# clearmatics/libff

Measured on AMD Instinct MI355X. Metric: G1 MSM throughput (scalar-muls/sec), higher is better.
Workload: dtype u32

## Files before the change

### libff_amd/csrc/group_vtable.h

```cpp
#pragma once
#include <hip/hip_runtime_api.h>
#include <stddef.h>
#include <stdint.h>
#include <stdlib.h>

namespace amdmsm {

enum out_form : int {
    OUT_JACOBIAN = 0,
    OUT_LIBFF = 1,
    OUT_AFFINE = 2,
};

struct sort_geom {
    int hb;
    int fb;
    uint32_t chunk_cap;
    uint32_t big_thresh;
    uint32_t big_cap;
    size_t big_words;
};
constexpr int SORT_HB_MAX = 10;
constexpr size_t SORT_COARSE_WORDS = ((size_t)1 << SORT_HB_MAX) + 1, SORT_CURSOR_WORDS = (size_t)1 << SORT_HB_MAX;
inline sort_geom sort_geometry(size_t n, int c, int W) {
// ... 98 lines not shown
    int fr_words;
    int el_words;
    int fq_words;
    int fr_bits;
    int projective;
    int reduce_fold;
    int bucket_words;
    const uint32_t* fr_one_mont;
    const uint32_t* fr_modulus;
    int has_endomorphism;
    int coeff_a_nonzero;
    int glv_bound_log2_x1000;
    int prime_order;
    const uint32_t* glv_lambda;

    void (*import_bases)(hipStream_t, const uint32_t* src, size_t stride_words, int form_special,
                         size_t n, uint32_t* dst_affine);
    void (*export_affine)(hipStream_t, const uint32_t* src_affine, size_t n, uint32_t* dst_xyz);
    void (*gen_bases_seq)(hipStream_t, unsigned long long first, size_t n, uint32_t* dst_affine);
    void (*endo_points)(hipStream_t, const uint32_t* bases_affine, size_t n, uint32_t* out);
    void (*precompute_table)(hipStream_t, const uint32_t* bases_affine, size_t n, int c, int D, uint32_t* tmp,
                             uint32_t* table);
    void (*ffi_decode_points)(hipStream_t, const uint32_t* src_be, size_t n, uint32_t* dst_affine, uint32_t* status);
    void (*ffi_decode_scalars)(hipStream_t, const uint32_t* src_be, size_t n, uint32_t* dst_plain, uint32_t* status);
    void (*ffi_encode_point)(hipStream_t, const uint32_t* src_xyz_affine, uint32_t* dst_be);
    void (*disk_decode)(hipStream_t, const uint32_t* src, size_t n, uint32_t* dst_affine);
    void (*disk_decode_compressed)(hipStream_t, const uint32_t* src, size_t n, uint32_t* dst_affine, uint32_t* status);
    void (*disk_encode)(hipStream_t, const uint32_t* src_affine, size_t n, uint32_t* dst);
    void (*disk_encode_compressed)(hipStream_t, const uint32_t* src_affine, size_t n, uint32_t* dst);

    void (*scalar_stats)(hipStream_t, const uint32_t* scalars, size_t n, int mont, uint32_t* stats);
    void (*scalar_bits)(hipStream_t, const void* scalars, int kind, size_t n, int mont, uint32_t* out_bits);
    void (*gather_scalars)(hipStream_t, const uint32_t* shared, size_t shared_n, const uint32_t* index, size_t offset,
                           uint32_t* flag, size_t n, uint32_t* out);
    void (*count)(hipStream_t, const uint32_t* scalars, size_t n, int mont, int c, int W, uint32_t* counts);
    void (*scatter)(hipStream_t, const uint32_t* scalars, size_t n, int mont, int c, int W, uint32_t* cursor,
                    uint32_t* lists, size_t list_stride);
    void (*sort)(hipStream_t, const sort_src& src, size_t n, int mont, int c, int W, const sort_bufs& bufs, int mode);
    int (*sort_top_window)(int mode, int mont, int c, int W, size_t columns, int* tb);

    void (*accumulate)(hipStream_t, const uint32_t* ends, const uint32_t* lists, size_t list_stride,
                       const uint32_t* bases_affine, uint32_t* buckets, uint32_t* part_first, uint32_t* part_last,
                       uint32_t* cont_bucket, int W, uint32_t B, uint32_t S, uint32_t T, const uint32_t* endo_points,
                       size_t n_real, int overlap);
    size_t (*accumulate_resident_lanes)(int overlap);
    int accumulate_overlap_ok;
    void (*accumulate_fixup)(hipStream_t, const uint32_t* ends, uint32_t* buckets, uint32_t* part_first,
                             const uint32_t* part_last, const uint32_t* cont_bucket, uint32_t* queue, int W,
                             uint32_t B, uint32_t S, uint32_t T);

    void (*reduce_segments)(hipStream_t, const uint32_t* buckets, int W, uint32_t B, uint32_t L, uint32_t* out);
    void (*sum_butterfly)(hipStream_t, const uint32_t* in, int W, uint32_t M, uint32_t* out);
    void (*sum_block)(hipStream_t, const uint32_t* in, int W, uint32_t M, uint32_t* out);
    void (*reduce_rowcol)(hipStream_t, const uint32_t* buckets, int W, uint32_t B, int c, uint32_t q_row, uint32_t q_col,
                          uint32_t* rc, uint32_t* planes, uint32_t* out);
    void (*horner)(hipStream_t, const uint32_t* window_sums, int W, int c, int form, const uint32_t* init,
                   uint32_t* out);
    void (*horner_batch)(hipStream_t, const uint32_t* window_sums, int k, int W, int c, int form, uint32_t* const* outs);
    void (*sum_points)(hipStream_t, const uint32_t* pts, int k, int form, uint32_t* out);

    void (*fixed_base_exp)(hipStream_t, const uint32_t* g_xyz, int scalar_size, int window, const uint32_t* scalars,
                           size_t n, int mont, const uint32_t* coeff, int form, uint32_t* gouter, uint32_t* table,
                           uint32_t* table_aff, int build_table, uint32_t* out);

    int smv_entries;
    void (*smv_table)(hipStream_t, const uint32_t* bases_affine, size_t n, uint32_t* tmp, uint32_t* table);
    void (*smv_ladder)(hipStream_t, const uint32_t* table, size_t n, const uint32_t* scalars, int mont, int form, uint32_t* out);

    int seg_windows, seg_digit_stride;
    void (*seg_digits)(hipStream_t, const uint32_t* scalars, size_t n, int mont, uint32_t* digits);
    void (*seg_accumulate)(hipStream_t, const uint32_t* table, size_t nt, const uint32_t* digits, const uint32_t* slices,
                           size_t n_slices, uint32_t* sums);
    void (*seg_fold)(hipStream_t, const uint32_t* sums, const uint32_t* seg_first, size_t m, uint32_t* winsum);
    void (*seg_horner)(hipStream_t, const uint32_t* winsum, size_t m, int form, uint32_t* out);

    int fold_digit_stride;
    void (*fold_digits)(hipStream_t, const uint32_t* scalars_host, int k, int mont, int glv, int W, uint32_t* digits);
    void (*fold_ladder)(hipStream_t, const uint32_t* tables, size_t n, const uint32_t* digits, int rows, int glv, int W,
                        int form, uint32_t* out);

    void (*fft_gather)(hipStream_t, const uint32_t* in_affine, size_t b0, size_t cn, int rsh, uint32_t* dst_affine);
    void (*fft_butterfly)(hipStream_t, const uint32_t* table, size_t cn, const uint32_t* in_affine, size_t b0, int rsh,
                          const uint32_t* twiddles, int mont, size_t half, uint32_t* out);

    void (*field_op)(hipStream_t, int op, const uint32_t* a, const uint32_t* b, uint32_t* out, size_t n);
    void (*group_op)(hipStream_t, int op, const uint32_t* a, const uint32_t* b, uint32_t* out, size_t n, int form);
    void (*digits)(hipStream_t, const uint32_t* scalars, size_t n, int mont, int c, int W, int32_t* out);
    void (*glv_digits)(hipStream_t, const uint32_t* scalars, size_t n, int mont, int c, int W, int32_t* out);
    void (*mul_bench)(hipStream_t, uint32_t* inout, size_t nthreads, int iters, int inline_variant);
    void (*madd_bench)(hipStream_t, const uint32_t* pts_affine, uint32_t* out_xyz, size_t nthreads, int iters,
                       int inline_variant);

    void (*field_probe)(hipStream_t, int impl, int op, const uint32_t* a, const uint32_t* b, const uint32_t* c,
                        const uint32_t* d, uint32_t* out, uint32_t* flag, size_t n);
    void (*xyzz_probe)(hipStream_t, int impl, int op, const uint32_t* acc, const uint32_t* pt, uint32_t* out, size_t n);
};
constexpr int FOLD_MAX_K = 8;
constexpr size_t FOLD_DIGIT_BYTES = 2048;

enum {
    FPROBE_MUL = 0, FPROBE_SQR = 1, FPROBE_ADD = 2, FPROBE_SUB = 3, FPROBE_NEG = 4, FPROBE_INV = 5, FPROBE_DBL = 6,
    FPROBE_CNEG = 7,
    FPROBE_HALF = 8, FPROBE_TO_MONT = 9, FPROBE_FROM_MONT = 10,
    FPROBE_SQRT = 11,
    FPROBE_MUL_LZ = 16, FPROBE_SQR_LZ = 17, FPROBE_SUB_LZ = 18, FPROBE_ADD_LZ = 19, FPROBE_NEG_LZ = 20,
    FPROBE_MUL_SUB_MUL_LZ = 21,
    FPROBE_IS_ZERO_LZ = 22,
// ... 18 lines not shown
```

### libff_amd/csrc/msm_group.hip

```cpp
#include "curve_params.h"
#include "ec.cuh"
#include "fp2h.cuh"
#include "group_vtable.h"
#include "wide.cuh"
#include "wide28.cuh"
#include "rr.cuh"

#include <algorithm>
#include <cstdio>
#include <vector>
#include <type_traits>

#ifndef AMDMSM_GROUP
#error "compile with -DAMDMSM_GROUP=<group traits> -DAMDMSM_VT=<vtable getter name>"
#endif

namespace amdmsm {
template <bool I>
struct ec_coeff_a<Fp<AMDMSM_GROUP::fq, I>> {
    static constexpr int value = AMDMSM_GROUP::DEG == 1 ? AMDMSM_GROUP::COEFF_A : 0;
};
template <int NR, bool I>
struct ec_coeff_a<Fp2<AMDMSM_GROUP::fq, NR, I>> {
    static constexpr int value = AMDMSM_GROUP::DEG == 2 ? AMDMSM_GROUP::COEFF_A : 0;
// ... 1832 lines not shown
        jac_add(p, p, x);
    }
    wave_group_sum_r(p, RED_FOLD);
    if (lane < (uint32_t)RED_LANES) store_jac(part + wave * XYZW, p);
    __syncthreads();
    if (wave != 0) return;
    const uint32_t jw = lane / RED_LANES;
    if (jw < nw) load_jac(p, part + jw * XYZW); else jac_set_inf(p);
    uint32_t G = 1;
    while (G < nw) G <<= 1;
    wave_group_sum_r(p, G);
    if (lane < (uint32_t)RED_LANES) store_jac(planes + ((size_t)w * c + k) * XYZW, p);
}

__global__ void __launch_bounds__(SUMW_THREADS) k_plane_sums_wide(const uint32_t* __restrict__ rc, int W, int c, int h,
                                                                  uint32_t* __restrict__ planes) {
    __shared__ uint32_t buf[2][SUMW_SLOTS * XYZW];
    __builtin_amdgcn_s_setprio(3);
    const uint32_t w = blockIdx.x / (uint32_t)c, k = blockIdx.x % (uint32_t)c;
    const uint32_t C = 1u << h, R = (1u << (c - 1)) >> h, NP = R + 1 + C;
    const bool from_cols = k < (uint32_t)h;
    const uint32_t* src = rc + ((size_t)w * NP + (from_cols ? R + 1 : 0)) * XYZW;
    const uint32_t bit = from_cols ? k : k - (uint32_t)h;
    const bool top = k == (uint32_t)c - 1;
    const uint32_t M = top ? 1u : (from_cols ? C : R) / 2;
    constexpr uint32_t NLANES = SUMW_THREADS / RED_LANES, NWAVES = SUMW_THREADS / 64;
    const uint32_t i0 = threadIdx.x / RED_LANES, wave = threadIdx.x >> 6;
    Jac<ER> p, x;
    jac_set_inf(p);
    for (uint32_t i = i0; i < M; i += NLANES) {
        const uint32_t idx = top ? R : (((i >> bit) << (bit + 1)) | (1u << bit) | (i & ((1u << bit) - 1u)));
        load_jac(x, src + (size_t)idx * XYZW);
        jac_add(p, p, x);
    }
    wave_group_sum_r(p, 4);
    if ((i0 & 3u) == 0) store_jac(buf[0] + (size_t)(i0 >> 2) * XYZW, p);
    __syncthreads();
    const WideEnv<FQ> env = wide_env<FQ>();
    uint32_t K = ((M < NLANES ? M : NLANES) + 3) / 4;
    int cur = 0;
    while (K > 1) {
        const uint32_t pairs = K / 2;
        for (uint32_t q = wave; q < pairs; q += NWAVES) {
            const uint32_t* a = buf[cur] + (size_t)(2 * q) * XYZW;
            sum_wide_add(env, a, a + XYZW, buf[cur ^ 1] + (size_t)q * XYZW);
        }
        __syncthreads();
        cur ^= 1;
        K = pairs;
    }
    for (uint32_t t = threadIdx.x; t < (uint32_t)XYZW; t += SUMW_THREADS) planes[((size_t)w * c + k) * XYZW + t] = buf[cur][t];
}

template <class P, bool I>
AMDMSM_DEV typename std::enable_if<(P::N < 16), void>::type horner_chain(Jac<Fp<P, I>>& res,
                                                                         const uint32_t* __restrict__ window_sums, int W,
                                                                         int c, const uint32_t* __restrict__ init) {
    const WideEnv<P> env = wide_env<P>();
    auto load = [&](const uint32_t* p, uint32_t& X, uint32_t& Y, uint32_t& Z) {
        X = env.valid ? p[env.j] : 0u;
        Y = env.valid ? p[EW + env.j] : 0u;
        Z = env.valid ? p[2 * EW + env.j] : 0u;
    };
    uint32_t X, Y, Z, X2, Y2, Z2;
    int w = W - 1;
    if (init) {
        load(init, X, Y, Z);
    } else {
        load(window_sums + (size_t)w * XYZW, X, Y, Z);
        --w;
    }
    for (; w >= 0; --w) {
        if (!wide_is_zero(Z)) {
            if constexpr (GP::COEFF_A != 0) for (int i = 0; i < c; ++i) jac_dbl_wide<P, GP::COEFF_A>(env, X, Y, Z);
            else if (c >= 4) jac_dbl_run28<P>(env, X, Y, Z, c);
            else for (int i = 0; i < c; ++i) jac_dbl_wide<P>(env, X, Y, Z);
        }
        load(window_sums + (size_t)w * XYZW, X2, Y2, Z2);
        jac_add_wide<P, GP::COEFF_A>(env, X, Y, Z, X2, Y2, Z2);
    }
    wide_to_packed(res.x, X);
    wide_to_packed(res.y, Y);
    wide_to_packed(res.z, Z);
}
template <class P, bool I>
AMDMSM_DEV typename std::enable_if<(P::N >= 16 && P::N < 32), void>::type horner_chain(
    Jac<Fp<P, I>>& res, const uint32_t* __restrict__ window_sums, int W, int c, const uint32_t* __restrict__ init) {
    using F = WideFq<P>;
    const WideEnv<P> env = wide_env<P>();
    auto load = [&](const uint32_t* p, uint32_t& X, uint32_t& Y, uint32_t& Z) {
        X = env.valid ? p[env.j] : 0u;
        Y = env.valid ? p[EW + env.j] : 0u;
        Z = env.valid ? p[2 * EW + env.j] : 0u;
    };
    uint32_t X, Y, Z, X2, Y2, Z2;
    int w = W - 1;
    if (init) {
        load(init, X, Y, Z);
    } else {
        load(window_sums + (size_t)w * XYZW, X, Y, Z);
        --w;
    }
    for (; w >= 0; --w) {
        if (!wide_is_zero(Z)) {
            if (c >= 4) jac_dbl_run28<P>(env, X, Y, Z, c);
            else for (int i = 0; i < c; ++i) jac_dbl_wide2<P>(env, X, Y, Z);
// ... 94 lines not shown
inline bool horner_lazy() {
    static const bool on = HORNER_LAZY_OK && !(getenv("AMDMSM_HORNER_LAZY") && atoi(getenv("AMDMSM_HORNER_LAZY")) == 0);
    return on;
}

__global__ void __launch_bounds__(64) k_horner(const uint32_t* __restrict__ window_sums, int W, int c, int form,
                                               const uint32_t* __restrict__ init, uint32_t* __restrict__ out) {
    __builtin_amdgcn_s_setprio(3);
    Jac<E> res;
    horner_chain(res, window_sums, W, c, init);
    if (threadIdx.x == 0) store_out(out, res, form);
}
template <class EE = E>
__global__ void __launch_bounds__(64) k_horner_lazy(const uint32_t* __restrict__ window_sums, int W, int c, int form,
                                                    const uint32_t* __restrict__ init, uint32_t* __restrict__ out) {
    __builtin_amdgcn_s_setprio(3);
    Jac<EE> res;
    horner_chain_lazy(res, window_sums, W, c, init);
    if (threadIdx.x == 0) store_out(out, res, form);
}

constexpr int WH_MAX_GROUPS = 6;
__global__ void __launch_bounds__(64 * WH_MAX_GROUPS) k_window_horner(const uint32_t* __restrict__ planes, int c,
                                                                       uint32_t* __restrict__ out) {
    __shared__ uint32_t grp[WH_MAX_GROUPS * XYZW];
    __builtin_amdgcn_s_setprio(3);
    const int wave = (int)(threadIdx.x >> 6), ng = (c + 3) / 4;
    Jac<E> res;
    if (wave < ng) {
        const int k0 = 4 * wave, cnt = (c - k0 < 4) ? c - k0 : 4;
        horner_chain(res, planes + ((size_t)blockIdx.x * c + k0) * XYZW, cnt, 1, nullptr);
        if ((threadIdx.x & 63u) == 0) store_jac(grp + wave * XYZW, res);
    }
    __syncthreads();
    if (wave != 0) return;
    horner_chain(res, grp, ng, 4, nullptr);
    if (threadIdx.x == 0) store_jac(out + (size_t)blockIdx.x * XYZW, res);
}
template <class EE = E>
__global__ void __launch_bounds__(64 * WH_MAX_GROUPS) k_window_horner_lazy(const uint32_t* __restrict__ planes, int c,
                                                                            uint32_t* __restrict__ out) {
    __shared__ uint32_t grp[WH_MAX_GROUPS * XYZW];
    __builtin_amdgcn_s_setprio(3);
    const int wave = (int)(threadIdx.x >> 6), ng = (c + 3) / 4;
    Jac<EE> res;
    if (wave < ng) {
        const int k0 = 4 * wave, cnt = (c - k0 < 4) ? c - k0 : 4;
        horner_chain_lazy(res, planes + ((size_t)blockIdx.x * c + k0) * XYZW, cnt, 1, nullptr);
        if ((threadIdx.x & 63u) == 0) store_jac(grp + wave * XYZW, res);
    }
    __syncthreads();
    if (wave != 0) return;
    horner_chain_lazy(res, grp, ng, 4, nullptr);
    if (threadIdx.x == 0) store_jac(out + (size_t)blockIdx.x * XYZW, res);
}

struct horner_outs {
    uint32_t* p[8];
};
__global__ void __launch_bounds__(64) k_horner_batch(const uint32_t* __restrict__ window_sums, int W, int c, int form,
                                                     horner_outs outs) {
    __builtin_amdgcn_s_setprio(3);
    Jac<E> res;
    horner_chain(res, window_sums + (size_t)blockIdx.x * W * XYZW, W, c, nullptr);
    uint32_t* out = outs.p[0];
#pragma unroll
    for (int j = 1; j < 8; ++j) out = (blockIdx.x == (unsigned)j) ? outs.p[j] : out;
    if (threadIdx.x == 0) store_out(out, res, form);
}
template <class EE = E>
__global__ void __launch_bounds__(64) k_horner_batch_lazy(const uint32_t* __restrict__ window_sums, int W, int c, int form,
                                                          horner_outs outs) {
    __builtin_amdgcn_s_setprio(3);
    Jac<EE> res;
    horner_chain_lazy(res, window_sums + (size_t)blockIdx.x * W * XYZW, W, c, nullptr);
    uint32_t* out = outs.p[0];
#pragma unroll
    for (int j = 1; j < 8; ++j) out = (blockIdx.x == (unsigned)j) ? outs.p[j] : out;
    if (threadIdx.x == 0) store_out(out, res, form);
}

__global__ void __launch_bounds__(64) k_sum_points(const uint32_t* __restrict__ pts, int k, int form,
                                                   uint32_t* __restrict__ out) {
    Jac<E> res;
    if (k <= 0) jac_set_inf(res);
    else horner_chain(res, pts, k, 0, nullptr);
    if (threadIdx.x == 0) store_out(out, res, form);
}

constexpr int IMPORT_K = 32;

__global__ void __launch_bounds__(TPB) k_import_bases(const uint32_t* __restrict__ src, size_t stride_words,
                                                      int form_special, size_t n, uint32_t* __restrict__ dst) {
    if (form_special) {
        const size_t i = gtid();
        if (i >= n) return;
        const uint32_t* q = src + i * stride_words;
        Aff<E> a;
        E z;
        el_load(a.x, q);
        el_load(a.y, q + EW);
        el_load(z, q + 2 * EW);
        if (el_is_zero(z)) {
            el_zero(a.x);
            el_zero(a.y);
        }
// ... 1041 lines not shown

__global__ void __launch_bounds__(TPB) k_seg_fold(const uint32_t* __restrict__ sums, const uint32_t* __restrict__ seg_first,
                                                  size_t lanes, uint32_t* __restrict__ winsum) {
    const size_t lane = gtid();
    if (lane >= lanes) return;
    const size_t seg = lane / SMV_DIGITS;
    const uint32_t w = (uint32_t)(lane - seg * SMV_DIGITS);
    Xyzz<E> acc, x;
    xyzz_set_inf(acc);
#pragma unroll 1
    for (uint32_t sl = seg_first[seg]; sl < seg_first[seg + 1]; ++sl) {
        load_xyzz(x, sums + ((size_t)sl * SMV_DIGITS + w) * ZZW);
        xyzz_add(acc, acc, x);
    }
    Jac<E> r;
    xyzz_to_jac(r, acc);
    store_jac(winsum + lane * XYZW, r);
}

__global__ void __launch_bounds__(64) k_seg_horner(const uint32_t* __restrict__ winsum, int form, uint32_t* __restrict__ out) {
    Jac<E> res;
    horner_chain(res, winsum + (size_t)blockIdx.x * SMV_DIGITS * XYZW, SMV_DIGITS, SMV_W, nullptr);
    if (threadIdx.x == 0) store_out(out + (size_t)blockIdx.x * XYZW, res, form);
}
template <class EE = E>
__global__ void __launch_bounds__(64) k_seg_horner_lazy(const uint32_t* __restrict__ winsum, int form, uint32_t* __restrict__ out) {
    Jac<EE> res;
    horner_chain_lazy(res, winsum + (size_t)blockIdx.x * SMV_DIGITS * XYZW, SMV_DIGITS, SMV_W, nullptr);
    if (threadIdx.x == 0) store_out(out + (size_t)blockIdx.x * XYZW, res, form);
}

template <bool OK> struct horner_lazy_el { using type = E; };
template <bool OK = HORNER_LAZY_OK>
void launch_horner(hipStream_t st, const uint32_t* window_sums, int W, int c, int form, const uint32_t* init, uint32_t* out) {
    if constexpr (OK) {
        if (horner_lazy()) {
            hipLaunchKernelGGL(k_horner_lazy<typename horner_lazy_el<OK>::type>, dim3(1), dim3(64), 0, st, window_sums, W, c, form, init, out);
            return;
        }
    }
    hipLaunchKernelGGL(k_horner, dim3(1), dim3(64), 0, st, window_sums, W, c, form, init, out);
}
template <bool OK = HORNER_LAZY_OK>
void launch_horner_batch(hipStream_t st, const uint32_t* window_sums, int k, int W, int c, int form, const horner_outs& o) {
    if constexpr (OK) {
        if (horner_lazy()) {
            hipLaunchKernelGGL(k_horner_batch_lazy<typename horner_lazy_el<OK>::type>, dim3((unsigned)k), dim3(64), 0, st, window_sums, W, c, form, o);
            return;
        }
    }
    hipLaunchKernelGGL(k_horner_batch, dim3((unsigned)k), dim3(64), 0, st, window_sums, W, c, form, o);
}
template <bool OK = HORNER_LAZY_OK>
void launch_window_horner(hipStream_t st, const uint32_t* planes, int W, int c, uint32_t* out) {
    const dim3 threads((unsigned)(64 * ((c + 3) / 4)));
    if constexpr (OK) {
        if (horner_lazy()) {
            hipLaunchKernelGGL(k_window_horner_lazy<typename horner_lazy_el<OK>::type>, dim3((unsigned)W), threads, 0, st, planes, c, out);
            return;
        }
    }
    hipLaunchKernelGGL(k_window_horner, dim3((unsigned)W), threads, 0, st, planes, c, out);
}
template <bool OK = HORNER_LAZY_OK>
void launch_seg_horner(hipStream_t st, const uint32_t* winsum, size_t m, int form, uint32_t* out) {
    if constexpr (OK) {
        if (horner_lazy()) {
            hipLaunchKernelGGL(k_seg_horner_lazy<typename horner_lazy_el<OK>::type>, dim3((unsigned)m), dim3(64), 0, st, winsum, form, out);
            return;
        }
    }
    hipLaunchKernelGGL(k_seg_horner, dim3((unsigned)m), dim3(64), 0, st, winsum, form, out);
}

static_assert(2 * FOLD_MAX_K * SMV_DS <= (int)FOLD_DIGIT_BYTES, "the digit rows fit the buffer the engine sets aside");
struct alignas(16) fold_scalars {
    uint32_t w[FOLD_MAX_K * FRW];
};

__global__ void __launch_bounds__(64) k_fold_digits(const fold_scalars sc, int k, int mont, int glv, int W,
                                                    uint32_t* __restrict__ digits) {
    const int j = (int)threadIdx.x;
    if (j >= k) return;
    uint32_t s[FRW];
    load_scalar(s, sc.w, (size_t)j, mont);
    uint32_t word = 0;
    auto put = [&](int row, int w, int32_t d) { put_digit_byte(digits + row * (SMV_DS / 4), word, w, W, d); };
    if (glv) {
        if constexpr (GP::HAS_ENDO) for_each_glv_digit(s, SMV_W, W, [&](int h, int w, int32_t d) { put(2 * j + h, w, d); });
    } else {
        for_each_signed_digit(s, SMV_W, W, [&](int w, int32_t d) { put(j, w, d); });
    }
}

__global__ void __launch_bounds__(TPB) k_fold_ladder(const uint32_t* __restrict__ tables, size_t n,
                                                     const uint32_t* __restrict__ digits, int rows, int glv, int W,
                                                     int form, uint32_t* __restrict__ out) {
    const size_t i = gtid();
    if (i >= n) return;
    int top = -1;
#pragma unroll 1
    for (int q = (W + 3) / 4 - 1; q >= 0 && top < 0; --q) {
        uint32_t any = 0;
#pragma unroll 1
        for (int r = 0; r < rows; ++r) any |= digits[r * (SMV_DS / 4) + q];
        if (any) top = 4 * q + (31 - __clz((int)any)) / 8;
    }
    const signed char* dg = (const signed char*)digits;
    Xyzz<E> acc;
    xyzz_set_inf(acc);
    Aff<E> e;
#pragma unroll 1
    for (int w = top; w >= 0; --w) {
        if (w != top) {
#pragma unroll 1
// ... 264 lines not shown
#else
    hipLaunchKernelGGL(k_accumulate, dim3(blocks_for((size_t)W * T * ACC_LANES)), dim3(TPB), dyn_lds, st, ends, lists,
                       list_stride, bases, buckets, part_first, part_last, cont_bucket, W, B, S, T, endo_pts,
                       endo_pts ? (uint32_t)n_real : 0x80000000u, sync_waves);
#endif
}
void l_endo_points(hipStream_t st, const uint32_t* bases, size_t n, uint32_t* out) {
    if (!n) return;
    hipLaunchKernelGGL(k_endo_points, dim3(blocks_for(n * 2 * GP::DEG)), dim3(TPB), 0, st, bases, n, out);
}
void l_glv_digits(hipStream_t st, const uint32_t* scalars, size_t n, int mont, int c, int W, int32_t* out) {
    if (!n) return;
    hipLaunchKernelGGL(k_glv_digits, dim3(blocks_for(n)), dim3(TPB), 0, st, scalars, n, mont, c, W, out);
}
size_t l_accumulate_resident_lanes(int overlap) {
    auto query = [](size_t dyn_lds) {
        int dev = 0, cus = 256, blocks = 0;
        if (hipGetDevice(&dev) == hipSuccess) (void)hipDeviceGetAttribute(&cus, hipDeviceAttributeMultiprocessorCount, dev);
        if (hipOccupancyMaxActiveBlocksPerMultiprocessor(&blocks, k_accumulate, TPB, dyn_lds) != hipSuccess || blocks <= 0) blocks = 4;
        return (size_t)cus * (size_t)blocks * TPB / ACC_LANES;
    };
    static const size_t lanes = query(0);
    static const size_t lanes_overlap = (AMDMSM_OVERLAP_OK && ACC_OVERLAP_LDS) ? query(ACC_OVERLAP_LDS) : lanes;
    return overlap ? lanes_overlap : lanes;
}
void l_accumulate_fixup(hipStream_t st, const uint32_t* ends, uint32_t* buckets, uint32_t* part_first,
                        const uint32_t* part_last, const uint32_t* cont_bucket, uint32_t* queue, int W, uint32_t B,
                        uint32_t S, uint32_t T) {
    const unsigned fix_blocks = blocks_for((size_t)W * T * RED_LANES, 64);
    const unsigned compact_blocks = T / FIX_BLOCK >= 2 ? (unsigned)(W * (T / FIX_BLOCK - 1)) : 0u;
    hipLaunchKernelGGL(k_accumulate_fixup, dim3(fix_blocks + compact_blocks), dim3(64), 0, st, ends, part_first,
                       part_last, cont_bucket, buckets, queue, W, B, S, T, fix_blocks);
    const size_t lanes = (size_t)W * T;
    const size_t cap_mid = fixup_queue_cap_mid(lanes) / (RED_FOLD / MID_G) + 1, cap_long = fixup_queue_cap_long(lanes);
    const unsigned mid_blocks = (unsigned)(cap_mid < 8192 ? cap_mid : 8192), long_blocks = (unsigned)(cap_long < 2048 ? cap_long : 2048);
    hipLaunchKernelGGL(k_accumulate_fixup_queue, dim3(mid_blocks + long_blocks), dim3(64), 0, st, ends,
                       part_first, part_last, cont_bucket, buckets, queue, mid_blocks, lanes, B, S, T);
}
void l_reduce_segments(hipStream_t st, const uint32_t* buckets, int W, uint32_t B, uint32_t L, uint32_t* out) {
    hipLaunchKernelGGL(k_reduce_segments, dim3(blocks_for((size_t)W * (B / L) * RED_LANES, 64)), dim3(64), 0, st, buckets, W, B,
                       L, out);
}
void l_sum_butterfly(hipStream_t st, const uint32_t* in, int W, uint32_t M, uint32_t* out) {
    hipLaunchKernelGGL(k_sum_butterfly, dim3(blocks_for((size_t)W * M * RED_LANES, 64)), dim3(64), 0, st, in, W, M, out);
}
void l_sum_block(hipStream_t st, const uint32_t* in, int W, uint32_t M, uint32_t* out) {
    if (M >= 8 && M * RED_LANES <= (uint32_t)SUMW_THREADS && (M & (M - 1)) == 0) {
        hipLaunchKernelGGL(k_sum_block_wide, dim3(W), dim3(SUMW_THREADS), 0, st, in, W, M, out);
        return;
    }
    const unsigned threads = (unsigned)((M * RED_LANES + 63) / 64 * 64);
    hipLaunchKernelGGL(k_sum_block, dim3(W), dim3(threads), 0, st, in, W, M, out);
}
void l_reduce_rowcol(hipStream_t st, const uint32_t* buckets, int W, uint32_t B, int c, uint32_t q_row, uint32_t q_col,
                     uint32_t* rc, uint32_t* planes, uint32_t* out) {
    const int h = c / 2;
    const uint32_t C = 1u << h, R = B >> h;
    auto fit = [](uint32_t len, uint32_t q) {
        if (q < 1) q = 1;
        while (q & (q - 1)) q &= q - 1;
        if (q > len) q = len;
        while (len / q > RED_FOLD) q <<= 1;
        return q;
    };
    q_row = fit(C, q_row);
    q_col = fit(R, q_col);
    const size_t row_lanes = (size_t)W * (R + 1) * (C / q_row) * RED_LANES, col_lanes = (size_t)W * C * (R / q_col) * RED_LANES;
    const unsigned row_blocks = blocks_for(row_lanes, 64), col_blocks = blocks_for(col_lanes, 64);
    hipLaunchKernelGGL(k_bucket_sums, dim3(row_blocks + col_blocks), dim3(64), 0, st, buckets, W, B, h, q_row, q_col, row_blocks, rc);
    const uint32_t maxm = (C > R ? C : R) / 2;
    static const bool wide_planes = !(getenv("AMDMSM_PLANES_WIDE") && atoi(getenv("AMDMSM_PLANES_WIDE")) == 0);
    if (maxm >= 8 && wide_planes) {
        hipLaunchKernelGGL(k_plane_sums_wide, dim3((unsigned)(W * c)), dim3(SUMW_THREADS), 0, st, rc, W, c, h, planes);
    } else {
        unsigned threads = (unsigned)((maxm * RED_LANES + 63) / 64 * 64);
        threads = threads < 64 ? 64 : (threads > 256 ? 256 : threads);
        hipLaunchKernelGGL(k_plane_sums, dim3((unsigned)(W * c)), dim3(threads), 0, st, rc, W, c, h, planes);
    }
    launch_window_horner(st, planes, W, c, out);
}
void l_horner(hipStream_t st, const uint32_t* window_sums, int W, int c, int form, const uint32_t* init, uint32_t* out) {
    launch_horner(st, window_sums, W, c, form, init, out);
}
void l_horner_batch(hipStream_t st, const uint32_t* window_sums, int k, int W, int c, int form, uint32_t* const* outs) {
    horner_outs o = {};
    for (int j = 0; j < k && j < 8; ++j) o.p[j] = outs[j];
    launch_horner_batch(st, window_sums, k, W, c, form, o);
}
void l_sum_points(hipStream_t st, const uint32_t* pts, int k, int form, uint32_t* out) {
    hipLaunchKernelGGL(k_sum_points, dim3(1), dim3(64), 0, st, pts, k, form, out);
}
void l_gen_bases_seq(hipStream_t st, unsigned long long first, size_t n, uint32_t* dst) {
    if (!n) return;
    hipLaunchKernelGGL(k_gen_bases_seq, dim3(blocks_for(n)), dim3(TPB), 0, st, first, n, dst);
}
void l_export_affine(hipStream_t st, const uint32_t* src, size_t n, uint32_t* dst) {
    if (!n) return;
    hipLaunchKernelGGL(k_export_affine, dim3(blocks_for(n)), dim3(TPB), 0, st, src, n, dst);
}
void l_ffi_decode_points(hipStream_t st, const uint32_t* src, size_t n, uint32_t* dst, uint32_t* status) {
    if (!n) return;
    hipLaunchKernelGGL(k_ffi_decode_points, dim3(blocks_for(n)), dim3(TPB), 0, st, src, n, dst, status);
}
void l_ffi_decode_scalars(hipStream_t st, const uint32_t* src, size_t n, uint32_t* dst, uint32_t* status) {
    if (!n) return;
    hipLaunchKernelGGL(k_ffi_decode_scalars, dim3(blocks_for(n)), dim3(TPB), 0, st, src, n, dst, status);
}
void l_ffi_encode_point(hipStream_t st, const uint32_t* src_xyz, uint32_t* dst) {
    hipLaunchKernelGGL(k_ffi_encode_point, dim3(1), dim3(64), 0, st, src_xyz, dst);
}
void l_disk_decode(hipStream_t st, const uint32_t* src, size_t n, uint32_t* dst) {
    if (!n) return;
    hipLaunchKernelGGL(k_disk_decode, dim3(blocks_for(n)), dim3(TPB), 0, st, src, n, dst);
}
void l_disk_decode_compressed(hipStream_t st, const uint32_t* src, size_t n, uint32_t* dst, uint32_t* status) {
    if (!n) return;
    hipLaunchKernelGGL(k_disk_decode_compressed, dim3(blocks_for(n, 64)), dim3(64), 0, st, src, n, dst, status);
}
constexpr size_t DISK_ENCODE_BLOCKS = 8192;
void l_disk_encode(hipStream_t st, const uint32_t* src, size_t n, uint32_t* dst) {
    if (!n) return;
    const unsigned blocks = (unsigned)std::min<size_t>((n + TPB - 1) / TPB, DISK_ENCODE_BLOCKS);
    hipLaunchKernelGGL(k_disk_encode, dim3(blocks), dim3(TPB), 0, st, src, n, dst);
}
void l_disk_encode_compressed(hipStream_t st, const uint32_t* src, size_t n, uint32_t* dst) {
    if (!n) return;
    const unsigned blocks = (unsigned)std::min<size_t>((n + TPB - 1) / TPB, DISK_ENCODE_BLOCKS);
    hipLaunchKernelGGL(k_disk_encode_compressed, dim3(blocks), dim3(TPB), 0, st, src, n, dst);
}
#if AMDMSM_ACC_RR
template <class G>
bool launch_fb_exp_rr(hipStream_t st, const uint32_t* table_aff, const uint32_t* scalars, size_t n, int mont, const uint32_t* coeff,
// ... 169 lines not shown
```

### libff_amd/csrc/wide28.cuh

```cuda
#pragma once
#include "wide.cuh"

namespace amdmsm {

template <int NW>
struct cbig {
    uint32_t w[NW];
};
template <int NW>
constexpr bool cb_ge(const cbig<NW>& a, const cbig<NW>& b) {
    for (int i = NW - 1; i >= 0; --i) {
        if (a.w[i] != b.w[i]) return a.w[i] > b.w[i];
    }
    return true;
}
template <int NW>
constexpr cbig<NW> cb_sub(const cbig<NW>& a, const cbig<NW>& b) {
    cbig<NW> r{};
    uint64_t borrow = 0;
    for (int i = 0; i < NW; ++i) {
        const uint64_t d = (uint64_t)a.w[i] - b.w[i] - borrow;
        r.w[i] = (uint32_t)d;
        borrow = (d >> 32) & 1u;
    }
// ... 245 lines not shown
    np = __ballot(n != v.pj);
}
template <int ROW>
AMDMSM_DEV bool row_zero28(unsigned long long nz, unsigned long long np) {
    return ((nz >> (16 * ROW)) & 0xffffull) == 0ull || ((np >> (16 * ROW)) & 0xffffull) == 0ull;
}

template <class P>
AMDMSM_DEV void jac_add_28(const Env28<P, 10>& v, uint32_t sub4, uint32_t& X1, uint32_t& Y1, uint32_t& Z1, uint32_t X2,
                           uint32_t Y2, uint32_t Z2) {
    const uint32_t row = (threadIdx.x & 63u) >> 4;
    const bool r0 = row == 0, r1 = row == 1, r2 = row == 2;
    unsigned long long nz, np;
    uint32_t r = mul28(v, r1 ? Z2 : Z1, r0 ? Z1 : Z2);
    exact28(v, r, nz, np);
    const bool inf1 = row_zero28<0>(nz, np), inf2 = row_zero28<1>(nz, np);
    if (inf2) {
        if (inf1) Z1 = 0u;
        return;
    }
    if (inf1) {
        X1 = X2;
        Y1 = Y2;
        Z1 = Z2;
        return;
    }
    const uint32_t z1z1 = from_row(r, 0), z2z2 = from_row(r, 1), z1z2 = from_row(r, 2);
    r = mul28(v, r0 ? X1 : (r1 ? X2 : (r2 ? Z2 : Z1)), (r0 || r2) ? z2z2 : z1z1);
    const uint32_t u1 = from_row(r, 0), u2 = from_row(r, 1), t1 = from_row(r, 2), t2 = from_row(r, 3);
    const uint32_t h = carry28(v, u2 + sub4 - u1), h2 = h + h;
    r = mul28(v, r0 ? Y1 : (r1 ? Y2 : (r2 ? h2 : z1z2)), r0 ? t1 : (r1 ? t2 : (r2 ? h2 : h)));
    exact28(v, r, nz, np);
    const bool hzero = row_zero28<2>(nz, np);
    const uint32_t s1 = from_row(r, 0), s2 = from_row(r, 1), ii = from_row(r, 2), zh = from_row(r, 3);
    const uint32_t d = carry28(v, s2 + sub4 - s1), rr = d + d;
    if (hzero) {
        exact28(v, mul28(v, rr, v.cout), nz, np);
        if (row_zero28<0>(nz, np)) {
            jac_dbl_28<P>(v, X1, Y1, Z1);
            exact28(v, mul28(v, Z1, v.cout), nz, np);
            if (row_zero28<0>(nz, np)) Z1 = 0u;
            return;
        }
    }
    r = mul28(v, r0 ? h : (r1 ? u1 : rr), r2 ? rr : ii);
    const uint32_t J = from_row(r, 0), V = from_row(r, 1), R2 = from_row(r, 2);
    X1 = sub28_16(v, R2, J + V + V);
    r = mul28(v, r0 ? rr : s1, r0 ? sub28_32(v, V, X1) : J);
    const uint32_t sj = from_row(r, 1);
    Y1 = sub28_16(v, from_row(r, 0), sj + sj);
    Z1 = hzero ? 0u : zh + zh;
}

template <class P, int NR>
struct WideFq2_28 {
    static constexpr int HEAD = 20;
    using V = Env28<P, HEAD>;
    static AMDMSM_DEV uint32_t mul(const V& v, uint32_t a, uint32_t b) {
        const uint32_t row = (threadIdx.x & 63u) >> 4;
        const bool r2 = row == 2, odd = (row & 1u) != 0;
        const uint32_t sa = a + row_swap(a), sb = b + row_swap(b);
        const uint32_t r = mul28(v, r2 ? sa : a, r2 ? sb : b);
        const uint32_t v0 = from_row(r, 0), v1 = from_row(r, 1), v2 = from_row(r, 2);
        const uint32_t nv1 = NR == -1 ? v1 : (v1 << 2) + v1;
        return carry28(v, (odd ? v2 : v0) + v.q16 - (odd ? v0 + v1 : nv1));
    }
    static AMDMSM_DEV uint32_t sqr(const V& v, uint32_t a) {
        if constexpr (NR != -1) {
            return mul(v, a, a);
        } else {
            const uint32_t row = (threadIdx.x & 63u) >> 4;
            const uint32_t sw = row_swap(a);
            const uint32_t s = a + sw, d = carry28(v, a + v.q512 - sw);
            const uint32_t r = mul28(v, row == 2 ? s : a, row == 2 ? d : sw);
            const uint32_t c0 = from_row(r, 2), x = from_row(r, 0);
            return (row & 1u) ? x + x : c0;
        }
    }
};
template <class P, int NR>
AMDMSM_DEV void jac_dbl_28q(const Env28<P, 20>& v, uint32_t& X, uint32_t& Y, uint32_t& Z) {
    using F = WideFq2_28<P, NR>;
    const uint32_t XX = F::sqr(v, X), B = F::sqr(v, Y), YZ = F::mul(v, Y, Z);
    const uint32_t B2 = carry28(v, B + B), E3 = carry28(v, XX + XX + XX);
    const uint32_t C4 = F::sqr(v, B2), XB2 = F::mul(v, X, B2);
    const uint32_t C8 = carry28(v, C4 + C4), D = carry28(v, XB2 + XB2);
    X = carry28(v, F::sqr(v, E3) + v.q128 - carry28(v, D + D));
    const uint32_t t = F::mul(v, E3, carry28(v, D + v.q256 - X));
    Y = carry28(v, t + v.q64 - C8);
    Z = carry28(v, YZ + YZ);
}
template <class P, int NR>
AMDMSM_DEV void jac_dbl_run28q(const WideEnv<P>& e, uint32_t& X, uint32_t& Y, uint32_t& Z, int c) {
    const Env28<P, 20> v = env28<P, 20>(e);
    uint32_t X28 = to28(v, X), Y28 = to28(v, Y), Z28 = to28(v, Z);
    for (int i = 0; i < c; ++i) jac_dbl_28q<P, NR>(v, X28, Y28, Z28);
    X = from28(v, X28);
    Y = from28(v, Y28);
    Z = from28(v, Z28);
}

}
```

Measured before the change: 662.1 million.

## Add lazy 28-bit plane-sum kernel with split halves and two-set window Horner

Result: no change. 666.4 million (median of 6 runs) (+0.6%).

```diff
diff --git a/libff_amd/csrc/group_vtable.h b/libff_amd/csrc/group_vtable.h
--- a/libff_amd/csrc/group_vtable.h
+++ b/libff_amd/csrc/group_vtable.h
@@ -174,7 +174,7 @@
     void (*reduce_segments)(hipStream_t, const uint32_t* buckets, int W, uint32_t B, uint32_t L, uint32_t* out);
     void (*sum_butterfly)(hipStream_t, const uint32_t* in, int W, uint32_t M, uint32_t* out);
     void (*sum_block)(hipStream_t, const uint32_t* in, int W, uint32_t M, uint32_t* out);
-    void (*reduce_rowcol)(hipStream_t, const uint32_t* buckets, int W, uint32_t B, int c, uint32_t q_row, uint32_t q_col,
+    void (*reduce_rowcol)(hipStream_t, uint32_t* buckets, int W, uint32_t B, int c, uint32_t q_row, uint32_t q_col,
                           uint32_t* rc, uint32_t* planes, uint32_t* out);
     void (*horner)(hipStream_t, const uint32_t* window_sums, int W, int c, int form, const uint32_t* init,
                    uint32_t* out);
diff --git a/libff_amd/csrc/msm_group.hip b/libff_amd/csrc/msm_group.hip
--- a/libff_amd/csrc/msm_group.hip
+++ b/libff_amd/csrc/msm_group.hip
@@ -1908,6 +1908,39 @@
     for (uint32_t t = threadIdx.x; t < (uint32_t)XYZW; t += SUMW_THREADS) planes[((size_t)w * c + k) * XYZW + t] = buf[cur][t];
 }
 
+constexpr int PLZ_WAVES = 16, PLZ_THREADS = 64 * PLZ_WAVES, PLZ_SLOTS = 256;
+template <class P>
+__global__ void __launch_bounds__(PLZ_THREADS) k_plane_sums_lazy(const uint32_t* __restrict__ rc, int W, int c, int h, int halves,
+                                                                 uint32_t* __restrict__ planes, uint32_t* __restrict__ planes_hi) {
+    __shared__ uint32_t slots[PLZ_SLOTS * SLOT28];
+    __builtin_amdgcn_s_setprio(3);
+    const uint32_t plane = blockIdx.x / (uint32_t)halves, g = blockIdx.x % (uint32_t)halves;
+    const uint32_t w = plane / (uint32_t)c, k = plane % (uint32_t)c;
+    const uint32_t C = 1u << h, R = (1u << (c - 1)) >> h, NP = R + 1 + C;
+    const bool from_cols = k < (uint32_t)h;
+    const uint32_t* src = rc + ((size_t)w * NP + (from_cols ? R + 1 : 0)) * XYZW;
+    const uint32_t bit = from_cols ? k : k - (uint32_t)h;
+    const bool top = k == (uint32_t)c - 1;
+    const uint32_t M = top ? 1u : (from_cols ? C : R) / 2;
+    const uint32_t share = (M + (uint32_t)halves - 1u) / (uint32_t)halves, first = g * share;
+    const uint32_t cnt = first >= M ? 0u : (M - first < share ? M - first : share);
+    uint32_t* out = (g ? planes_hi : planes) + (size_t)plane * XYZW;
+    if (cnt == 0) {
+        if (threadIdx.x < (uint32_t)XYZW) out[threadIdx.x] = 0u;
+        return;
+    }
+    const uint32_t wave = threadIdx.x >> 6;
+    const Env28<P, 10> v = env28<P, 10>(wide_env<P>());
+    const uint32_t sub4 = tab28_sel(A28<P>::SUB4, v.j);
+    slots28_fill<P, PLZ_SLOTS / PLZ_WAVES>(v, slots, cnt, wave, PLZ_WAVES, [&](uint32_t i) {
+        const uint32_t n = first + i;
+        const uint32_t idx = top ? R : (((n >> bit) << (bit + 1)) | (1u << bit) | (n & ((1u << bit) - 1u)));
+        return src + (size_t)idx * XYZW;
+    });
+    slots28_sum<P>(v, sub4, slots, cnt, wave, PLZ_WAVES);
+    if (wave == 0) slot28_write_out<P>(v, slots, out);
+}
+
 template <class P, bool I>
 AMDMSM_DEV typename std::enable_if<(P::N < 16), void>::type horner_chain(Jac<Fp<P, I>>& res,
                                                                          const uint32_t* __restrict__ window_sums, int W,
@@ -2108,6 +2141,31 @@
     __syncthreads();
     if (wave != 0) return;
     horner_chain_lazy(res, grp, ng, 4, nullptr);
+    if (threadIdx.x == 0) store_jac(out + (size_t)blockIdx.x * XYZW, res);
+}
+
+template <class EE = E>
+__global__ void __launch_bounds__(128 * WH_MAX_GROUPS) k_window_horner_lazy2(const uint32_t* __restrict__ planes,
+                                                                             const uint32_t* __restrict__ planes_hi, int c,
+                                                                             uint32_t* __restrict__ out) {
+    __shared__ uint32_t grp[2 * WH_MAX_GROUPS * XYZW];
+    __shared__ uint32_t part[2 * XYZW];
+    __builtin_amdgcn_s_setprio(3);
+    const int wave = (int)(threadIdx.x >> 6), ng = (c + 3) / 4;
+    const int set = wave >= ng ? 1 : 0, j = wave - set * ng;
+    uint32_t* mine = grp + set * WH_MAX_GROUPS * XYZW;
+    Jac<EE> res;
+    const int k0 = 4 * j, cnt = (c - k0 < 4) ? c - k0 : 4;
+    horner_chain_lazy(res, (set ? planes_hi : planes) + ((size_t)blockIdx.x * c + k0) * XYZW, cnt, 1, nullptr);
+    if ((threadIdx.x & 63u) == 0) store_jac(mine + j * XYZW, res);
+    __syncthreads();
+    if (j == 0) {
+        horner_chain_lazy(res, mine, ng, 4, nullptr);
+        if ((threadIdx.x & 63u) == 0) store_jac(part + set * XYZW, res);
+    }
+    __syncthreads();
+    if (wave != 0) return;
+    horner_chain_lazy(res, part, 2, 0, nullptr);
     if (threadIdx.x == 0) store_jac(out + (size_t)blockIdx.x * XYZW, res);
 }
 
@@ -3255,15 +3313,55 @@
     hipLaunchKernelGGL(k_horner_batch, dim3((unsigned)k), dim3(64), 0, st, window_sums, W, c, form, o);
 }
 template <bool OK = HORNER_LAZY_OK>
-void launch_window_horner(hipStream_t st, const uint32_t* planes, int W, int c, uint32_t* out) {
+void launch_window_horner(hipStream_t st, const uint32_t* planes, const uint32_t* planes_hi, int W, int c, uint32_t* out) {
     const dim3 threads((unsigned)(64 * ((c + 3) / 4)));
     if constexpr (OK) {
+        if (planes_hi) {
+            hipLaunchKernelGGL(k_window_horner_lazy2<typename horner_lazy_el<OK>::type>, dim3((unsigned)W), dim3(2 * threads.x), 0, st, planes, planes_hi, c, out);
+            return;
+        }
         if (horner_lazy()) {
             hipLaunchKernelGGL(k_window_horner_lazy<typename horner_lazy_el<OK>::type>, dim3((unsigned)W), threads, 0, st, planes, c, out);
             return;
         }
     }
     hipLaunchKernelGGL(k_window_horner, dim3((unsigned)W), threads, 0, st, planes, c, out);
+}
+constexpr uint32_t PLZ_SPLIT_MIN = 64;
+inline unsigned stream_cus(hipStream_t st) {
+    thread_local int dev_seen = -1;
+    thread_local unsigned cus_seen = 0;
+    int dev = 0, cus = 0;
+    if (hipStreamGetDevice(st, &dev) != hipSuccess && hipGetDevice(&dev) != hipSuccess) {
+        (void)hipGetLastError();
+        return 0;
+    }
+    if (dev == dev_seen) return cus_seen;
+    if (hipDeviceGetAttribute(&cus, hipDeviceAttributeMultiprocessorCount, dev) != hipSuccess || cus <= 0) {
+        (void)hipGetLastError();
+        return 0;
+    }
+    dev_seen = dev;
+    return cus_seen = (unsigned)cus;
+}
+template <bool OK> struct plane_lazy_fq { using type = FQ; };
+template <bool OK = HORNER_LAZY_OK>
+bool launch_plane_sums_lazy(hipStream_t st, const uint32_t* rc, int W, int c, int h, uint32_t maxm, uint32_t* planes,
+                            uint32_t* scratch, size_t scratch_words, const uint32_t** planes_hi) {
+    if constexpr (OK) {
+        static const int lazy = getenv("AMDMSM_PLANES_LAZY") ? atoi(getenv("AMDMSM_PLANES_LAZY")) : 1;
+        static const int split = getenv("AMDMSM_PLANES_SPLIT") ? atoi(getenv("AMDMSM_PLANES_SPLIT")) : 1;
+        if (lazy == 0 || !horner_lazy() || maxm > (uint32_t)PLZ_SLOTS) return false;
+        const unsigned nplanes = (unsigned)(W * c);
+        const bool room = (size_t)nplanes * XYZW <= scratch_words;
+        const bool two = split != 0 && maxm >= PLZ_SPLIT_MIN && room && (split == 2 || 2 * nplanes <= stream_cus(st));
+        if (!two && lazy != 2) return false;
+        const int halves = two ? 2 : 1;
+        hipLaunchKernelGGL(k_plane_sums_lazy<typename plane_lazy_fq<OK>::type>, dim3(nplanes * halves), dim3(PLZ_THREADS), 0, st, rc, W, c, h, halves, planes, scratch);
+        if (two) *planes_hi = scratch;
+        return true;
+    }
+    return false;
 }
 template <bool OK = HORNER_LAZY_OK>
 void launch_seg_horner(hipStream_t st, const uint32_t* winsum, size_t m, int form, uint32_t* out) {
@@ -3634,7 +3732,7 @@
     const unsigned threads = (unsigned)((M * RED_LANES + 63) / 64 * 64);
     hipLaunchKernelGGL(k_sum_block, dim3(W), dim3(threads), 0, st, in, W, M, out);
 }
-void l_reduce_rowcol(hipStream_t st, const uint32_t* buckets, int W, uint32_t B, int c, uint32_t q_row, uint32_t q_col,
+void l_reduce_rowcol(hipStream_t st, uint32_t* buckets, int W, uint32_t B, int c, uint32_t q_row, uint32_t q_col,
                      uint32_t* rc, uint32_t* planes, uint32_t* out) {
     const int h = c / 2;
     const uint32_t C = 1u << h, R = B >> h;
@@ -3651,15 +3749,17 @@
     const unsigned row_blocks = blocks_for(row_lanes, 64), col_blocks = blocks_for(col_lanes, 64);
     hipLaunchKernelGGL(k_bucket_sums, dim3(row_blocks + col_blocks), dim3(64), 0, st, buckets, W, B, h, q_row, q_col, row_blocks, rc);
     const uint32_t maxm = (C > R ? C : R) / 2;
+    const uint32_t* planes_hi = nullptr;
     static const bool wide_planes = !(getenv("AMDMSM_PLANES_WIDE") && atoi(getenv("AMDMSM_PLANES_WIDE")) == 0);
     if (maxm >= 8 && wide_planes) {
-        hipLaunchKernelGGL(k_plane_sums_wide, dim3((unsigned)(W * c)), dim3(SUMW_THREADS), 0, st, rc, W, c, h, planes);
+        if (!launch_plane_sums_lazy(st, rc, W, c, h, maxm, planes, buckets, (size_t)W * B * ZZS, &planes_hi))
+            hipLaunchKernelGGL(k_plane_sums_wide, dim3((unsigned)(W * c)), dim3(SUMW_THREADS), 0, st, rc, W, c, h, planes);
     } else {
         unsigned threads = (unsigned)((maxm * RED_LANES + 63) / 64 * 64);
         threads = threads < 64 ? 64 : (threads > 256 ? 256 : threads);
         hipLaunchKernelGGL(k_plane_sums, dim3((unsigned)(W * c)), dim3(threads), 0, st, rc, W, c, h, planes);
     }
-    launch_window_horner(st, planes, W, c, out);
+    launch_window_horner(st, planes, planes_hi, W, c, out);
 }
 void l_horner(hipStream_t st, const uint32_t* window_sums, int W, int c, int form, const uint32_t* init, uint32_t* out) {
     launch_horner(st, window_sums, W, c, form, init, out);
diff --git a/libff_amd/csrc/wide28.cuh b/libff_amd/csrc/wide28.cuh
--- a/libff_amd/csrc/wide28.cuh
+++ b/libff_amd/csrc/wide28.cuh
@@ -321,6 +321,61 @@
     Z1 = hzero ? 0u : zh + zh;
 }
 
+constexpr int SLOT28 = 48;
+AMDMSM_DEV void slot28_store_rows(uint32_t* slot, uint32_t r) {
+    const uint32_t lane = threadIdx.x & 63u;
+    if (lane < (uint32_t)SLOT28) slot[lane] = r;
+}
+AMDMSM_DEV void slot28_store(uint32_t* slot, uint32_t X, uint32_t Y, uint32_t Z) {
+    const uint32_t row = (threadIdx.x & 63u) >> 4;
+    slot28_store_rows(slot, row == 0 ? X : (row == 1 ? Y : Z));
+}
+AMDMSM_DEV void slot28_load(const uint32_t* slot, uint32_t& X, uint32_t& Y, uint32_t& Z) {
+    const uint32_t j = threadIdx.x & 15u;
+    X = slot[j];
+    Y = slot[16 + j];
+    Z = slot[32 + j];
+}
+template <class P, int SHARE, class REC>
+AMDMSM_DEV void slots28_fill(const Env28<P, 10>& v, uint32_t* slots, uint32_t M, uint32_t wave, uint32_t nwaves, REC rec) {
+    const uint32_t row = (threadIdx.x & 63u) >> 4;
+    uint32_t raw[SHARE];
+#pragma unroll
+    for (int t = 0; t < SHARE; ++t) {
+        const uint32_t i = wave + (uint32_t)t * nwaves;
+        raw[t] = (i < M && v.e.valid && row < 3u) ? rec(i)[row * (uint32_t)P::N + v.j] : 0u;
+    }
+#pragma unroll
+    for (int t = 0; t < SHARE; ++t) {
+        const uint32_t i = wave + (uint32_t)t * nwaves;
+        if (i < M) slot28_store_rows(slots + (size_t)i * SLOT28, to28(v, raw[t]));
+    }
+    __syncthreads();
+}
+template <class P>
+AMDMSM_DEV void slots28_sum(const Env28<P, 10>& v, uint32_t sub4, uint32_t* slots, uint32_t K, uint32_t wave, uint32_t nwaves) {
+    while (K > 1) {
+        const uint32_t half = (K + 1) / 2;
+        for (uint32_t q = wave; q < K - half; q += nwaves) {
+            uint32_t X1, Y1, Z1, X2, Y2, Z2;
+            slot28_load(slots + (size_t)q * SLOT28, X1, Y1, Z1);
+            slot28_load(slots + (size_t)(q + half) * SLOT28, X2, Y2, Z2);
+            jac_add_28<P>(v, sub4, X1, Y1, Z1, X2, Y2, Z2);
+            slot28_store(slots + (size_t)q * SLOT28, X1, Y1, Z1);
+        }
+        __syncthreads();
+        K = half;
+    }
+}
+template <class P>
+AMDMSM_DEV void slot28_write_out(const Env28<P, 10>& v, const uint32_t* slots, uint32_t* out) {
+    const uint32_t row = (threadIdx.x & 63u) >> 4;
+    uint32_t X, Y, Z;
+    slot28_load(slots, X, Y, Z);
+    const uint32_t r = from28(v, row == 0 ? X : (row == 1 ? Y : Z));
+    if (v.e.valid && row < 3u) out[row * (uint32_t)P::N + v.j] = r;
+}
+
 template <class P, int NR>
 struct WideFq2_28 {
     static constexpr int HEAD = 20;
```
